# thien/stereo.vision

Hardware: AMD Instinct MI355X
Metric: Mpoints/sec disparity→3D at 1024×544; achieved HBM GB/s vs peak (higher is better)
Workload: dtype u8->f32; 1 GPU; configs[2]: 4096/GPU x 1024x544, step 1, dense fp32 XYZ (K1); frames_per_gpu=4096, global_frames=4096, H=544, W=1024, step=1, grid_points_per_frame=555489, parallelism=frame-sharded x1; one process

## Files before the change

stereo.vision_amd/csrc/kernels/resident.hip:

```cpp
#include "../svx_launch.h"

namespace svx {

constexpr int kRMaxChunks = 256;
constexpr int kRBins = 1000;
constexpr int kRDN = 32;
constexpr int kRDxStride = 33;
constexpr int kRDyOff = kRDN * kRDxStride;
constexpr int kRTxGroup = 20;
constexpr int kRTyOff = 64 * kRTxGroup;
constexpr int kRDeltaWords = kRTyOff + 32 > kRDyOff + kRDN ? kRTyOff + 32 : kRDyOff + kRDN;

__device__ __forceinline__ uint32_t pk_max16(uint32_t a, uint32_t b) {
    typedef unsigned short us2 __attribute__((ext_vector_type(2)));
    return __builtin_bit_cast(uint32_t, __builtin_elementwise_max(__builtin_bit_cast(us2, a), __builtin_bit_cast(us2, b)));
}


template <int STEP, int QP, bool LC>
struct RCfg {
    static constexpr int QPL = QP;
    static constexpr int CW = 3 * STEP;
};
template <int STEP>
// ... 537 lines not shown
        uint32_t cw[QPL][RCfg<STEP, QP, LC>::CW];
        r_load_bgr<STEP, QP, LC>(fbgr, r.g, p, cw);
        __syncthreads();
        uint32_t pos0;
        const uint32_t wtotal = r_stage_colours_sel<STEP, QP, LC>(keep, cw, wstage, sh.dump + tid, pos0);
        for (uint32_t j = lane; j < wtotal; j += kWave) {
            const uint32_t bin = r_bin_sel(wstage[j]);
            wstage[j] = (int64_t)hist[bin] > (int64_t)p.hist_thr ? 1u : 0u;
        }
        uint32_t pos = pos0;
#pragma unroll
        for (int b = 0; b < 4 * QPL; ++b) {
            if (keep & (1u << b)) {
                if (!wstage[pos]) keep &= ~(1u << b);
                ++pos;
            }
        }
    }
    uint64_t cnt = 0, inc;
    const auto add = [](uint32_t a, uint32_t b) { return a + b; };
    if constexpr (LC) {
        cnt = (uint64_t)__builtin_popcount(keep);
        inc = (uint64_t)wave_scan_dpp((uint32_t)cnt, add);
    } else {
#pragma unroll
        for (int i = 0; i < QPL; ++i) cnt += (uint64_t)__builtin_popcount((keep >> (4 * i)) & 0xF) << (16 * i);
        inc = (uint64_t)wave_scan_dpp((uint32_t)cnt, add) | ((uint64_t)wave_scan_dpp((uint32_t)(cnt >> 32), add) << 32);
    }
    if (lane == 63) sh.wtot[wave] = inc;
    __syncthreads();
    uint64_t wbase = 0, tot = 0;
#pragma unroll
    for (int w = 0; w < 4; ++w) {
        const uint64_t v = sh.wtot[w];
        wbase += (w < wave) ? v : 0ull;
        tot += v;
    }
    const uint64_t excl = wbase + inc - cnt;
    const uint32_t T = LC ? (uint32_t)tot
                          : (uint32_t)((tot >> 0) & 0xFFFF) + (uint32_t)((tot >> 16) & 0xFFFF) +
                                (uint32_t)((tot >> 32) & 0xFFFF) + (uint32_t)((tot >> 48) & 0xFFFF);
    if (tid < (int)(running - flushed)) sh.stage[(flushed + tid) & (stage_of<QP>() - 1)] = sh.red[tid];
    if (T > (uint32_t)stage_of<QP>() - (running - flushed)) {
        p2_write<STEP, QP, LC>(sh.stage, flushed, running, oX, oY, oZ, oPxy, p);
        flushed = running;
        __syncthreads();
    }
    uint32_t rowbase = running;
    uint32_t olc = running + (uint32_t)excl;
    const uint32_t tyl = (LC && narrow) ? dl[kRTyOff + (((uint32_t)max(r.g.gy[0], 0) * STEP) & 31u)] : 0u;
    uint32_t bxm = 0u, bym = 0u;
#pragma unroll
    for (int i = 0; i < QPL; ++i) {
        uint32_t o = LC ? olc : rowbase + (uint32_t)((excl >> (16 * i)) & 0xFFFF);
        rowbase += (uint32_t)((tot >> (16 * i)) & 0xFFFF);
        const uint32_t gy = (uint32_t)max(r.g.gy[i], 0), y = gy * STEP;
        uint32_t dv[4], bx[4], by[4];
#pragma unroll
        for (int k = 0; k < 4; ++k) dv[k] = r_d<STEP, QP, LC>(r.dw[i], k);
        if (narrow && LC) {
            const uint32_t x0 = 4u * (uint32_t)r.g.q[0];
            const uint4 tw = *reinterpret_cast<const uint4*>(dl + (x0 >> 4) * kRTxGroup + 4 * i);
            const uint32_t t4[4] = {tw.x, tw.y, tw.z, tw.w};
#pragma unroll
            for (int k = 0; k < 4; ++k) {
                const uint32_t dd = min(dv[k] - (uint32_t)dlo, (uint32_t)kRDN - 1);
                bx[k] = (t4[k] >> dd) & 1u;
                by[k] = (tyl >> dd) & 1u;
            }
        } else if (narrow) {
#pragma unroll
            for (int k = 0; k < 4; ++k) {
                const uint32_t dd = min(dv[k] - (uint32_t)dlo, (uint32_t)kRDN - 1);
                const uint32_t x = (uint32_t)(4 * r.g.q[i] + k) * STEP;
                bx[k] = (dl[dd * kRDxStride + (x >> 5)] >> (x & 31)) & 1u;
                by[k] = (dl[kRDyOff + dd] >> (y & 31)) & 1u;
            }
        } else {
#pragma unroll
            for (int k = 0; k < 4; ++k) {
                const uint32_t x = (uint32_t)(4 * r.g.q[i] + k) * STEP;
                const uint32_t xw = min(x >> 5, (uint32_t)p.dx_words - 1);
                bx[k] = (bf.dxbits[dv[k] * p.dx_words + xw] >> (x & 31)) & 1u;
                by[k] = (bf.dybits[dv[k] * p.dy_words + (y >> 5)] >> (y & 31)) & 1u;
            }
        }
#pragma unroll
        for (int k = 0; k < 4; ++k) {
            const uint32_t bit = (keep >> (4 * i + k)) & 1u;
            *(bit ? &sh.stage[o & (stage_of<QP>() - 1)] : sh.dump + tid) =
                rdesc(dv[k], gy, (uint32_t)(4 * r.g.q[i] + k), bx[k], by[k]);
            o += bit;
            if constexpr (RB) {
                bxm |= bx[k] << (4 * i + k);
                bym |= by[k] << (4 * i + k);
            }
        }
        olc = o;
    }
    if constexpr (RB) {
        static_assert(!RB || (LC && STEP == 1 && QPL == 4), "the road bitmap needs lane-contiguous step-1 quads");
        rb_mark(sh, keep, bxm, bym, r.g.gy[0], 4 * r.g.q[0], bf.rb_Wu);
    }
    if (PF && more) p2_load<STEP, QP, LC>(r, c + 1, tid, fdisp, sh.crange, bf, p, true, next_run, fkb);
    __syncthreads();
    running += T;
    const uint32_t upto = more ? (running & ~31u) : running;
    if (tid < (int)(running - upto)) sh.red[tid] = sh.stage[(upto + tid) & (stage_of<QP>() - 1)];
    if (upto > flushed) {
        p2_write<STEP, QP, LC>(sh.stage, flushed, upto, oX, oY, oZ, oPxy, p);
        flushed = upto;
    }
}

template <int QP>
struct FusedShared {
    uint32_t hist[kRBins];
    uint32_t dirty[maxchunks_of<QP>() / 32];
    uint64_t wtot[4];
    uint32_t red[32];
    uint32_t stage[stage_of<QP>()];
    uint32_t dump[256];
    alignas(16) uint32_t crange[maxchunks_of<QP>() * 4];
    uint32_t dlt[kRDeltaWords];
    uint32_t cany[8];
    uint32_t rring[8 * 32];
    uint32_t rwrap[32];
};
static_assert(sizeof(FusedShared<4>) <= 32768, "5 workgroups per CU (160 KiB LDS), as many as 93 VGPRs allow");

template <int STEP, int QP, bool LC>
__device__ __forceinline__ void chunk_keepable_bits(FusedShared<QP>& sh, const FramePlane* Lp, const RParams& p) {
    constexpr int per = RCfg<STEP, QP, LC>::QPL * 256;
    const int c = threadIdx.x;
    bool k = false;
    const FramePlane L = *Lp;
    if (c < p.nchunks && L.valid) {
        const int gy0 = fastdiv40(c * per, p.Q_m40);
        const int gy1 = fastdiv40(min((c + 1) * per, p.frame_quads) - 1, p.Q_m40);
        k = rows_keepable(L, gy0, gy1, p.Wg, STEP);
    }
    const uint64_t m = __ballot(k);
    if (lane_id() == 0) {
        sh.cany[2 * (c >> 6)] = (uint32_t)m;
        sh.cany[2 * (c >> 6) + 1] = (uint32_t)(m >> 32);
    }
}

template <int QP>
__device__ __forceinline__ bool chunk_any(const FusedShared<QP>& sh, int c) {
    return __builtin_amdgcn_readfirstlane((sh.cany[c >> 5] >> (c & 31)) & 1u) != 0;
}

template <int STEP, int QP, bool LC, bool PF1 = false>
__device__ __forceinline__ void frame_pass1(int frame, FusedShared<QP>& sh, const PipeBuffers& bf,
                                            const RLean& L, const FramePlane* Lp,
                                            const RParams& p) {
    constexpr int WREGION = 64 * RCfg<STEP, QP, LC>::QPL * 4;
    const int tid = threadIdx.x, lane = lane_id(), wave = tid >> 6;
    const uint8_t* fdisp = bf.disp + (int64_t)frame * p.frame_px;
    const uint8_t* fbgr = bf.bgr + (int64_t)frame * p.frame_px * 3;
    uint32_t* wstage = sh.stage + wave * WREGION;
    for (int i = tid; i < kRBins; i += 256) sh.hist[i] = 0;
    if (tid < maxchunks_of<QP>() / 32) sh.dirty[tid] = 0;
    chunk_keepable_bits<STEP, QP, LC>(sh, Lp, p);
    __syncthreads();
    uint32_t nvalid = 0, nkept = 0;
    uint16_t* fkb = bf.kbits + (int64_t)frame * p.nchunks * 256;
    const int n1 = ablated(p.ablate, 128) ? 0 : p.nchunks;
    if constexpr (PF1) {
        P1Regs<STEP, QP, LC> r1;
        if (n1 > 0) p1_load<STEP, QP, LC>(r1, 0, tid, fdisp, fbgr, p, false, chunk_any(sh, 0));
        for (int c = 0; c < n1; ++c) {
            P1Regs<STEP, QP, LC> cur = r1;
            const bool any = chunk_any(sh, c);
            const uint32_t keep = any ? r_keep1<STEP, QP, LC>(cur.dw, cur.g, L, Lp, p.Wg) : 0u;
            if (c + 1 < n1) p1_load<STEP, QP, LC>(r1, c + 1, tid, fdisp, fbgr, p, true, chunk_any(sh, c + 1));
            p1_chunk<STEP, QP, LC>(cur, c, sh.hist, sh.dirty, sh.crange, wstage, sh.dump + tid, p, nvalid, nkept,
                               any, fkb, keep);
        }
    } else {
        for (int c = 0; c < n1; ++c) {
            P1Regs<STEP, QP, LC> r1;
            const bool any = chunk_any(sh, c);
            p1_load<STEP, QP, LC>(r1, c, tid, fdisp, fbgr, p, false, any);
            const uint32_t keep = any ? r_keep1<STEP, QP, LC>(r1.dw, r1.g, L, Lp, p.Wg) : 0u;
            p1_chunk<STEP, QP, LC>(r1, c, sh.hist, sh.dirty, sh.crange, wstage, sh.dump + tid, p, nvalid, nkept, any, fkb,
                               keep);
        }
    }
    nvalid = wave_sum(nvalid);
    nkept = wave_sum(nkept);
    if (lane == 0) {
        sh.red[wave] = nvalid;
        sh.red[4 + wave] = nkept;
    }
    __syncthreads();
}

template <int STEP, int QP, bool LC, bool PF, bool RB>
__device__ __forceinline__ void frame_pass2(int frame, FusedShared<QP>& sh, const PipeBuffers& bf,
                                            const RLean& L, const FramePlane* Lp,
                                            const RParams& p) {
    constexpr int WREGION = 64 * RCfg<STEP, QP, LC>::QPL * 4;
    const int tid = threadIdx.x, wave = tid >> 6;
    const uint8_t* fdisp = bf.disp + (int64_t)frame * p.frame_px;
    const uint8_t* fbgr = bf.bgr + (int64_t)frame * p.frame_px * 3;
    uint32_t* wstage = sh.stage + wave * WREGION;
    float* oX = bf.ox + (int64_t)frame * bf.ofs;
    float* oY = bf.oy + (int64_t)frame * bf.ofs;
    float* oZ = bf.oz + (int64_t)frame * bf.ofs;
    uint32_t* oPxy = bf.pxy + (int64_t)frame * bf.cap;
    uint32_t running = 0, flushed = 0;
    const int n2 = ablated(p.ablate, 256) ? 0 : p.nchunks;
    const auto run = [&](int c) {
        const uint4 cr = *reinterpret_cast<const uint4*>(sh.crange + 4 * c);
        return c + 1 == n2 || (cr.x | cr.y | cr.z | cr.w) != 0u;
    };
    const uint16_t* fkb = bf.kbits + (int64_t)frame * p.nchunks * 256;
    uint32_t* frb = RB ? bf.rbits + (int64_t)frame * bf.rb_H * 32 : nullptr;
    int rflushed = 0;
    if constexpr (RB) {
        sh.rring[tid] = 0u;
        if (tid < 32) sh.rwrap[tid] = 0u;
        __syncthreads();
    }
    constexpr int RPC = RB ? 4 : 1;
    P2Regs<STEP, QP, LC> r2;
    r2.staged = false;
    if (PF && n2 > 0) p2_load<STEP, QP, LC>(r2, 0, tid, fdisp, sh.crange, bf, p, false, run(0), fkb);
    for (int c = 0; c < n2; ++c) {
        if (!PF) p2_load<STEP, QP, LC>(r2, c, tid, fdisp, sh.crange, bf, p, c > 0, run(c), fkb);
        if (!run(c)) {
            if (PF) p2_load<STEP, QP, LC>(r2, c + 1, tid, fdisp, sh.crange, bf, p, true, run(c + 1), fkb);
            if constexpr (RB) rb_flush(sh, frb, rflushed, RPC * (c + 1) - 1, bf.rb_H);
            continue;
        }
        p2_chunk<STEP, QP, LC, PF, RB>(r2, c, c + 1 < n2, sh.hist, sh.dirty, sh, wstage, fdisp, fbgr, L, Lp, bf, oX, oY,
                                       oZ, oPxy,
                                       running, flushed, c + 1 < n2 && run(c + 1), fkb, p);
        if constexpr (RB) {
            if (c + 1 < n2) {
                rb_flush(sh, frb, rflushed, RPC * (c + 1) - 1, bf.rb_H);
            } else {
                while (rflushed < bf.rb_H) rb_flush(sh, frb, rflushed, min(rflushed + 8, bf.rb_H), bf.rb_H);
            }
        }
    }
    if (tid == 0) bf.counts[4 * (int64_t)frame + 2] = running;
}

template <int STEP, int QP, bool LC, bool PF, bool PF1, bool RB>
__device__ __forceinline__ void fused_body(const PipeBuffers& bf, const RParams& p,
                                           FusedShared<QP>& sh) {
    const int tid = threadIdx.x;
    const int frame = blockIdx.x;
    const FramePlane* Lp = bf.planes + (int64_t)frame * bf.plane_stride;
    const RLean L{Lp->al32, Lp->bb32, Lp->b032, Lp->tn32, Lp->g32};
    if (const uint32_t us = ablate_field(p.ablate, 20, 0xFFFu); us && blockIdx.x < 5 * 256) {
        const uint64_t t0 = wall_clock64(), wait = (uint64_t)(blockIdx.x >> 8) * us * 100u;
        while (wall_clock64() - t0 < wait) __builtin_amdgcn_s_sleep(32);
    }
    frame_pass1<STEP, QP, LC, PF1>(frame, sh, bf, L, Lp, p);
    __builtin_amdgcn_s_setprio(2);
    uint32_t* gh = bf.hist + (int64_t)frame * kBins;
    for (int b = tid; b < kBins; b += 256) gh[b] = b < kRBins ? sh.hist[b] : 0u;
    if (tid == 0) {
        int64_t* cn = bf.counts + 4 * (int64_t)frame;
        cn[0] = (int64_t)sh.red[0] + sh.red[1] + sh.red[2] + sh.red[3];
        cn[1] = (int64_t)sh.red[4] + sh.red[5] + sh.red[6] + sh.red[7];
    }
    frame_pass2<STEP, QP, LC, PF, RB>(frame, sh, bf, L, Lp, p);
}

template <int STEP, int QP, bool LC, bool PF, bool PF1 = false, bool RB = false>
__global__ __launch_bounds__(256) __attribute__((amdgpu_waves_per_eu(5))) void resident_fused_kernel(PipeBuffers bf, RParams p) {
    __shared__ FusedShared<QP> sh;
    fused_body<STEP, QP, LC, PF, PF1, RB>(bf, p, sh);
}

bool resident_supported(const KParams& p) {
    return (p.step == 1 || p.step == 2) && p.pitch <= 2048 && p.Hg <= 2048 &&
           resident_chunks_per_frame(p, 4) <= kRMaxChunks && p.frame_px * 3 < (1ll << 31);
}

static bool resident_lane_quads(const KParams& kp) {
    const char* v = svx_knob("SVX_RES_LC");
    const bool on = !(v && v[0] == '0');
    return on && kp.step == 1 && kp.Q % 4 == 0 && kp.W % 16 == 0 && kp.frame_px % 16 == 0;
}

bool resident_road_bits_supported(const KParams& p) {
    return resident_supported(p) && p.step == 1 && p.W == 1024 && p.Q == 256 && p.H <= 1024 && p.Hg >= 1 &&
           resident_lane_quads(p);
}

static RParams resident_params(const KParams& kp, int qpl) {
    RParams p;
    p.W = kp.W;
    p.Wg = kp.Wg;
    p.Q = kp.Q;
    p.pitch = kp.pitch;
    p.frame_quads = kp.frame_quads;
    p.nchunks = resident_chunks_per_frame(kp, qpl);
    p.drow = 256 * qpl / kp.Q;
    p.dq = 256 * qpl % kp.Q;
    p.hist_thr = kp.hist_thr;
    p.dx_words = kp.dx_words;
    p.dy_words = kp.dy_words;
    p.ablate = kp.ablate;
    p.Q_m40 = kp.Q_m40;
    p.frame_px = kp.frame_px;
    p.B32 = kp.B32;
    p.fB32 = kp.fB32;
    p.cw_hi = kp.cw_hi;
    p.cw_lo = kp.cw_lo;
    p.ch_hi = kp.ch_hi;
    p.ch_lo = kp.ch_lo;
    return p;
}

__global__ void store_plane_kernel(FramePlane v, FramePlane* __restrict__ dst) {
    if (threadIdx.x == 0) *dst = v;
}

hipError_t launch_store_plane(const FramePlane& v, FramePlane* dst, hipStream_t s) {
    hipLaunchKernelGGL(store_plane_kernel, dim3(1), dim3(64), 0, s, v, dst);
    return hipGetLastError();
}

hipError_t launch_pipeline_resident(const KParams& kp, const PipeBuffers& b, int frames,
                                    bool prefetch, hipStream_t s, bool prefetch1, const char** kname) {
    if (frames <= 0) return hipSuccess;
    if (!resident_supported(kp) || !b.planes) return hipErrorInvalidValue;
    const dim3 grid(frames), block(256);
// ... 35 lines not shown
```

stereo.vision_amd/csrc/kernels/sgbm.hip:

```cpp
#include <hip/hip_runtime.h>
#include <stdint.h>

#include <algorithm>
#include <type_traits>
#include <cstdlib>

#include "../svx_device.h"
#include "../svx_sgbm.h"
#include "../svx_wave.h"

namespace svx {
namespace {

constexpr int kMaxCost = 32767;
constexpr int kInt16Min = -32768;

__device__ __forceinline__ int lo16(uint32_t v) { return (int)(int16_t)(v & 0xFFFF); }
__device__ __forceinline__ int hi16(uint32_t v) { return (int)(int16_t)(v >> 16); }
__device__ __forceinline__ uint32_t pack16(int a, int b) { return (uint32_t)(uint16_t)a | ((uint32_t)(uint16_t)b << 16); }
__device__ __forceinline__ int sat16(int v) { return v < kInt16Min ? kInt16Min : (v > kMaxCost ? kMaxCost : v); }
__device__ __forceinline__ bool out16(int v) { return v < kInt16Min || v > kMaxCost; }

__device__ __forceinline__ int wave_min_i32(int v) {
    return wave_readlane(wave_scan(v, 0x7fffffff, [](int a, int b) { return min(a, b); }), 63);
// ... 412 lines not shown
                pk_step(cw, st, k.P1, k.P2, q);
                (q2vol + o)[lane] = q_byte_pk(q);
            } else {
                int L0, L1;
                path_step(cw0, cw1, st, k.P1, k.P2, L0, L1);
                (l2vol + o)[lane] = pack16(L0, L1);
            }
        }
#pragma unroll
        for (int u = 0; u < U; ++u) {
            ca[u] = na[u];
            cr[u] = nr[u];
        }
    }
    if (__any(st.ovf()) && lane == 0) atomicOr(flags + f, 1u);
}

template <int SH2C, bool DQ>
__global__ __launch_bounds__(256) void sgbm_vertical_ring_kernel(SgbmK k, const uint32_t* __restrict__ hvol,
                                                                   uint32_t* __restrict__ cvol,
                                                                   uint32_t* __restrict__ l2vol,
                                                                   uint8_t* __restrict__ q2vol,
                                                                   uint32_t* __restrict__ flags, int frames) {
    constexpr int RS = 2 * SH2C + 1;
    const int wpb = blockDim.x >> 6;
    const int cols_blocks = (k.width1 + wpb - 1) / wpb;
    const int f = blockIdx.x / cols_blocks;
    const int xi = (blockIdx.x - f * cols_blocks) * wpb + wave_uniform_id();
    if (f >= frames || xi >= k.width1) return;
    const uint32_t lane = lane_id();
    const int H = k.H;
    const size_t rs = (size_t)k.width1 * 64;
    const size_t base = (size_t)f * H * rs + (size_t)xi * 64;
    const uint32_t rs32 = (uint32_t)rs;
    const __amdgpu_buffer_rsrc_t rh = wave_rsrc(hvol + base, (size_t)H * rs * 4),
                                 rcv = wave_rsrc(cvol + base, (size_t)H * rs * 4), rq2 = wave_rsrc(q2vol + base, (size_t)H * rs);
    const auto hrow = [&](int r) { return bld32(rh, lane * 4, (uint32_t)min(r, H - 1) * rs32 * 4); };
    uint32_t drop[RS];
    int c0 = 0, c1 = 0;
#pragma unroll
    for (int kk = 0; kk <= SH2C; ++kk) {
        const uint32_t h = hrow(kk);
        const int sc = kk == 0 ? SH2C + 1 : 1;
        c0 += lo16(h) * sc;
        c1 += hi16(h) * sc;
        if (kk == 0) {
#pragma unroll
            for (int u = 0; u <= SH2C + 1; ++u) drop[u] = h;
        } else if (kk < SH2C) {
            drop[kk + SH2C + 1] = h;
        }
    }
    std::conditional_t<DQ, PathPk, PathState> st;
    const bool upd_col = xi > 0;
    uint32_t add[RS];
#pragma unroll
    for (int u = 0; u < RS; ++u) add[u] = hrow(u + SH2C);
    const auto vstep = [&](int u, int y) {
        if (y > 0 && upd_col && y + SH2C < H) {
            c0 += lo16(add[u]) - lo16(drop[u]);
            c1 += hi16(add[u]) - hi16(drop[u]);
        }
        drop[u] = add[u];
        const int cw0 = (int)(int16_t)c0, cw1 = (int)(int16_t)c1;
        const uint32_t cw = pack16(cw0, cw1);
        bst32(cw, rcv, lane * 4, (uint32_t)y * rs32 * 4);
        if constexpr (DQ) {
            uint32_t q;
            pk_step(cw, st, k.P1, k.P2, q);
            bst8(q_byte_pk(q), rq2, lane, (uint32_t)y * rs32);
        } else {
            int L0, L1;
            path_step(cw0, cw1, st, k.P1, k.P2, L0, L1);
            (l2vol + base + (size_t)y * rs)[lane] = pack16(L0, L1);
        }
    };
    int y0 = 0;
    for (; y0 + RS <= H; y0 += RS) {
        uint32_t nadd[RS];
#pragma unroll
        for (int u = 0; u < RS; ++u) nadd[u] = hrow(y0 + RS + u + SH2C);
#pragma unroll
        for (int u = 0; u < RS; ++u) vstep(u, y0 + u);
#pragma unroll
        for (int u = 0; u < RS; ++u) add[u] = nadd[u];
    }
#pragma unroll
    for (int u = 0; u < RS; ++u)
        if (y0 + u < H) vstep(u, y0 + u);
    if (__any(st.ovf()) && lane == 0) atomicOr(flags + f, 1u);
}

template <bool DQ>
__global__ __launch_bounds__(256) void sgbm_diag_kernel(SgbmK k, const uint32_t* __restrict__ cvol,
                                                          uint32_t* __restrict__ l1vol, uint32_t* __restrict__ l3vol,
                                                          uint8_t* __restrict__ q1vol, uint8_t* __restrict__ q3vol,
                                                          uint32_t* __restrict__ flags, int frames) {
    const int wpb = blockDim.x >> 6;
    const int npaths = k.width1 + k.H - 1;
    const int per_frame = 2 * npaths;
    const int gw = blockIdx.x * wpb + wave_uniform_id();
    const int f = gw / per_frame;
    if (f >= frames) return;
    int p = gw - f * per_frame;
    const int dir = p >= npaths;
    p -= dir * npaths;
    int xi, y;
    if (p < k.width1) {
        xi = p;
        y = 0;
    } else {
        xi = dir ? k.width1 - 1 : 0;
        y = p - k.width1 + 1;
    }
    const int len = min(k.H - y, dir ? xi + 1 : k.width1 - xi);
    const uint32_t lane = lane_id();
    const size_t rs = (size_t)k.width1 * 64;
    const size_t a0 = (size_t)f * k.H * rs + (size_t)y * rs + (size_t)xi * 64;
    const size_t step = dir ? rs - 64 : rs + 64;
    uint32_t* out = dir ? l3vol : l1vol;
    uint8_t* qout = dir ? q3vol : q1vol;
    const size_t span = (size_t)(len - 1) * step + 64;
    const __amdgpu_buffer_rsrc_t rc = wave_rsrc(cvol + a0, span * 4), rq = wave_rsrc(qout + a0, span);
    const uint32_t st32 = (uint32_t)step;
    const auto cell = [&](int t) { return bld32(rc, lane * 4, (uint32_t)min(t, len - 1) * st32 * 4); };
    std::conditional_t<DQ, PathPk, PathState> st;
    constexpr int U = kSgPf;
    uint32_t cc[U];
#pragma unroll
    for (int u = 0; u < U; ++u) cc[u] = cell(u);
    for (int t0 = 0; t0 < len; t0 += U) {
        uint32_t nc[U];
#pragma unroll
        for (int u = 0; u < U; ++u) nc[u] = cell(t0 + U + u);
#pragma unroll
        for (int u = 0; u < U; ++u) {
            const int t = t0 + u;
            if (t >= len) break;
            const size_t o = a0 + (size_t)t * step;
            if constexpr (DQ) {
                uint32_t q;
                pk_step(cc[u], st, k.P1, k.P2, q);
                bst8(q_byte_pk(q), rq, lane, (uint32_t)t * st32);
            } else {
                int L0, L1;
                path_step(lo16(cc[u]), hi16(cc[u]), st, k.P1, k.P2, L0, L1);
                (out + o)[lane] = pack16(L0, L1);
            }
        }
#pragma unroll
        for (int u = 0; u < U; ++u) cc[u] = nc[u];
    }
    if (__any(st.ovf()) && lane == 0) atomicOr(flags + f, 1u);
}


__host__ __device__ constexpr size_t sgbm_row_lds_per_wave(int W) { return ((size_t)6 * W + 3) & ~(size_t)3; }

template <bool DQ>
__global__ __launch_bounds__(256) void sgbm_row_kernel(SgbmK k, const uint32_t* __restrict__ cvol,
                                                         uint32_t* __restrict__ l1p, const uint32_t* __restrict__ l2vol,
                                                         const uint32_t* __restrict__ l3vol,
                                                         uint8_t* __restrict__ q0vol, const uint8_t* __restrict__ q1vol,
                                                         const uint8_t* __restrict__ q2vol,
                                                         const uint8_t* __restrict__ q3vol, int16_t* __restrict__ d16,
                                                         uint32_t* __restrict__ flags, int frames) {
    constexpr int U = kSgPf;
    extern __shared__ uint32_t rsm32[];
    const int wpb = blockDim.x >> 6, wave = wave_uniform_id();
    const int gw = blockIdx.x * wpb + wave;
    const int f = gw / k.H, y = gw - f * k.H;
    if (f >= frames) return;
    const int W = k.W;
    const uint32_t lane = lane_id();
    uint32_t* d2key = rsm32 + wave * (sgbm_row_lds_per_wave(W) / 4);
    int16_t* disp1 = reinterpret_cast<int16_t*>(d2key + W);
    const int INVALID = -kSgScale;
    for (int x = lane; x < W; x += 64) {
        disp1[x] = (int16_t)INVALID;
        d2key[x] = ~0u;
    }
    wave_lds_sync();
    const size_t rs = (size_t)k.width1 * 64;
    const size_t rb = ((size_t)f * k.H + y) * rs;
    const int n = k.width1;
    const auto at = [&](auto* vol, int xi) { return vol + rb + (size_t)xi * 64; };
    const __amdgpu_buffer_rsrc_t rc = wave_rsrc(cvol + rb, rs * 4), rq0 = wave_rsrc(q0vol + rb, rs),
                                 rq1 = wave_rsrc(q1vol + rb, rs), rq2 = wave_rsrc(q2vol + rb, rs),
                                 rq3 = wave_rsrc(q3vol + rb, rs);
    std::conditional_t<DQ, PathPk, PathState> sa, sb;
    {
        uint32_t cc[U], ca[U], cb[U], ce[U];
        const auto load = [&](int xi, uint32_t& c, uint32_t& a, uint32_t& b, uint32_t& e) {
            xi = min(xi, n - 1);
            if constexpr (DQ) {
                c = bld32(rc, lane * 4, (uint32_t)xi * 256);
            } else {
                c = at(cvol, xi)[lane];
                a = at(l1p, xi)[lane];
                b = at(l2vol, xi)[lane];
                e = at(l3vol, xi)[lane];
            }
        };
#pragma unroll
        for (int u = 0; u < U; ++u) load(u, cc[u], ca[u], cb[u], ce[u]);
        for (int x0 = 0; x0 < n; x0 += U) {
            uint32_t nc[U], na[U], nb[U], ne[U];
#pragma unroll
            for (int u = 0; u < U; ++u) load(x0 + U + u, nc[u], na[u], nb[u], ne[u]);
#pragma unroll
            for (int u = 0; u < U; ++u) {
                const int xi = x0 + u;
                if (xi >= n) break;
                if constexpr (DQ) {
                    uint32_t q;
                    pk_step(cc[u], sa, k.P1, k.P2, q);
                    bst8(q_byte_pk(q), rq0, lane, (uint32_t)xi * 64);
                } else {
                    int L0, L1;
                    path_step(lo16(cc[u]), hi16(cc[u]), sa, k.P1, k.P2, L0, L1);
                    const uint32_t pv = pack16(sat16(L0 + lo16(ca[u]) + lo16(cb[u]) + lo16(ce[u])),
                                               sat16(L1 + hi16(ca[u]) + hi16(cb[u]) + hi16(ce[u])));
                    __builtin_nontemporal_store(pv, at(l1p, xi) + lane);
                }
            }
#pragma unroll
            for (int u = 0; u < U; ++u) {
                cc[u] = nc[u];
                ca[u] = na[u];
                cb[u] = nb[u];
                ce[u] = ne[u];
            }
        }
    }
    {
        const int d0 = 2 * lane;
        uint32_t cc[U], cp[U];
        const auto load = [&](int j, uint32_t& c, uint32_t& pp) {
            const int xi = max(n - 1 - j, 0);
            if constexpr (DQ) {
                const uint32_t so = (uint32_t)xi * 64;
                c = bld32(rc, lane * 4, so * 4, true);
                pp = bld8(rq0, lane, so, true) | bld8(rq1, lane, so, true) << 8 | bld8(rq2, lane, so, true) << 16 |
                     bld8(rq3, lane, so, true) << 24;
            } else {
                c = at(cvol, xi)[lane];
                pp = at(l1p, xi)[lane];
            }
        };
#pragma unroll
        for (int u = 0; u < U; ++u) load(u, cc[u], cp[u]);
        for (int j0 = 0; j0 < n; j0 += U) {
            uint32_t nc[U], np[U];
#pragma unroll
            for (int u = 0; u < U; ++u) load(j0 + U + u, nc[u], np[u]);
            int gkey = -1, gnum = 0, gdv = 1;
#pragma unroll
            for (int u = 0; u < U; ++u) {
                const int xi = n - 1 - (j0 + u);
                if (xi < 0) break;
                int L0, L1, lm;
                uint32_t Lpk = 0;
                int P0, P1;
                if constexpr (DQ) {
                    uint32_t q;
                    Lpk = pk_l(cc[u], sb, k.P1, k.P2, q, lm);
                    L0 = lo16(Lpk);
                    L1 = hi16(Lpk);
                    P0 = sat16(4 * lo16(cc[u]) - (int)__builtin_amdgcn_sad_u8(cp[u] & 0x0F0F0F0Fu, 0u, 0u));
                    P1 = sat16(4 * hi16(cc[u]) - (int)__builtin_amdgcn_sad_u8((cp[u] >> 4) & 0x0F0F0F0Fu, 0u, 0u));
                } else {
                    lm = path_l(lo16(cc[u]), hi16(cc[u]), sb, k.P1, k.P2, L0, L1);
                    P0 = lo16(cp[u]);
                    P1 = hi16(cp[u]);
                }
                const int S0 = sat16(P0 + L0), S1 = sat16(P1 + L1);
                const int key = min(((S0 + 32768) << 7) | d0, ((S1 + 32768) << 7) | (d0 + 1));
                int wm, kmin;
                wave_min2_i32(lm, key, wm, kmin);
                if constexpr (DQ)
                    pk_commit(sb, cc[u], Lpk, wm);
                else
                    path_commit(sb, L0, L1, lm, wm);
                const int minS = (kmin >> 7) - 32768, best = kmin & 127;
                bool write = minS != kMaxCost;
                if (k.uniq > 0) {
                    const bool bad = (S0 * (100 - k.uniq) < minS * 100 && abs(best - d0) > 1) ||
                                     (S1 * (100 - k.uniq) < minS * 100 && abs(best - d0 - 1) > 1);
                    if (__any(bad)) write = false;
                }
                int num = 0, dv = 1;
                if (write && best > 0 && best < kSgD - 1) {
                    const uint32_t spk = pack16(S0, S1);
                    const uint32_t wm = (uint32_t)__builtin_amdgcn_readlane((int)spk, (best - 1) >> 1);
                    const uint32_t wp = (uint32_t)__builtin_amdgcn_readlane((int)spk, (best + 1) >> 1);
                    const int Sm = (best - 1) & 1 ? hi16(wm) : lo16(wm);
                    const int Sp = (best + 1) & 1 ? hi16(wp) : lo16(wp);
                    const int den = max(Sm + Sp - 2 * minS, 1);
                    num = (Sm - Sp) * kSgScale + den;
                    dv = den * 2;
                }
                if (write && lane == (uint32_t)u) {
                    gkey = kmin;
                    gnum = num;
                    gdv = dv;
                }
// ... 234 lines not shown
    t[threadIdx.x] = lut ? lut[threadIdx.x] : (uint8_t)threadIdx.x;
    __syncthreads();
    const int64_t per = (px + gridDim.x - 1) / gridDim.x;
    const int f = blockIdx.y;
    const int64_t p0 = blockIdx.x * per, p1 = min(px, p0 + per);
    const uint8_t* src = bgr + (size_t)f * px * 3;
    for (int64_t p = p0 + threadIdx.x; p < p1; p += blockDim.x) {
        const uint8_t* c = src + 3 * p;
        const int g = (t[c[0]] * 1868 + t[c[1]] * 9617 + t[c[2]] * 4899 + (1 << 13)) >> 14;
        grey[(size_t)f * px + p] = (uint8_t)g;
        atomicAdd(&h[g], 1u);
    }
    __syncthreads();
    if (h[threadIdx.x]) atomicAdd(hist + f * 256 + threadIdx.x, h[threadIdx.x]);
}

__global__ __launch_bounds__(256) void equalize_kernel(uint8_t* __restrict__ grey, int64_t px,
                                                         const uint32_t* __restrict__ hist) {
    __shared__ uint8_t lut[256];
    const int f = blockIdx.y;
    const uint32_t* h = hist + f * 256;
    if (threadIdx.x == 0) {
        int i = 0;
        while (i < 255 && !h[i]) ++i;
        if ((int64_t)h[i] == px) {
            for (int j = 0; j < 256; ++j) lut[j] = (uint8_t)i;
        } else {
            const float scale = 255.f / (float)(px - (int64_t)h[i]);
            int64_t sum = 0;
            lut[i] = 0;
            for (int j = i + 1; j < 256; ++j) {
                sum += h[j];
                const float v = __fmul_rn((float)sum, scale);
                const int r = (int)rintf(v);
                lut[j] = (uint8_t)(r < 0 ? 0 : r > 255 ? 255 : r);
            }
            for (int j = 0; j < i; ++j) lut[j] = 0;
        }
    }
    __syncthreads();
    uint8_t* g = grey + (size_t)f * px;
    for (int64_t p = (int64_t)blockIdx.x * blockDim.x + threadIdx.x; p < px; p += (int64_t)gridDim.x * blockDim.x)
        g[p] = lut[g[p]];
}

__global__ void synth_pair_kernel(uint8_t* __restrict__ left, uint8_t* __restrict__ right, int H, int W, int frames,
                                  int64_t first) {
    const int64_t i = (int64_t)blockIdx.x * blockDim.x + threadIdx.x;
    const int64_t px = (int64_t)H * W;
    const int64_t f = i / px;
    if (f >= frames) return;
    const int p = (int)(i - f * px);
    const int y = p / W, x = p - y * W;
    const int D = sgbm_pair_disparity(y);
    left[i] = sgbm_pair_texture(first + f, H, y, x);
    right[i] = sgbm_pair_texture(first + f, H, y, x + D);
}

__global__ void synth_bgr_pair_kernel(uint8_t* __restrict__ left, uint8_t* __restrict__ right, int H, int W,
                                      int frames, int64_t first) {
    const int64_t i = (int64_t)blockIdx.x * blockDim.x + threadIdx.x;
    const int64_t px = (int64_t)H * W;
    const int64_t f = i / px;
    if (f >= frames) return;
    const int p = (int)(i - f * px);
    const int y = p / W, x = p - y * W;
    const int D = sgbm_pair_disparity(y);
#pragma unroll
    for (int side = 0; side < 2; ++side) {
        const int u = side ? x + D : x;
        const int t = sgbm_pair_texture(first + f, H, y, u);
        const int j = sgbm_pair_texture(first + f + 0x4000000000ll, H, y, u);
        uint8_t* o = (side ? right : left) + 3 * i;
        o[0] = (uint8_t)t;
        o[1] = (uint8_t)min(255, t + (j & 31));
        o[2] = (uint8_t)max(0, t - ((j >> 3) & 31));
    }
}

__global__ __launch_bounds__(256) void copy_bgr_region_kernel(const uint8_t* __restrict__ src, int Hp, int Wp,
                                                              uint8_t* __restrict__ dst, int H, int W, int Wu,
                                                              const uint8_t* __restrict__ lut) {
    __shared__ uint8_t t[256];
    t[threadIdx.x] = lut ? lut[threadIdx.x] : (uint8_t)threadIdx.x;
    __syncthreads();
    const int row = blockIdx.x, f = blockIdx.y;
    const uint8_t* s = src + ((int64_t)f * Hp + row) * Wp * 3;
    uint8_t* d = dst + ((int64_t)f * H + row) * W * 3;
    for (int b = threadIdx.x; b < 3 * Wu; b += blockDim.x) d[b] = t[s[b]];
}

}

hipError_t launch_synth_bgr_pair(uint8_t* left, uint8_t* right, int H, int W, int frames, int64_t first,
                                 hipStream_t s) {
    const int64_t n = (int64_t)frames * H * W;
    hipLaunchKernelGGL(synth_bgr_pair_kernel, dim3((unsigned)((n + 255) / 256)), dim3(256), 0, s, left, right, H, W,
                       frames, first);
    return hipGetLastError();
}

hipError_t launch_copy_bgr_region(const uint8_t* src, int Hp, int Wp, uint8_t* dst, int H, int W, int Wu, int frames,
                                  hipStream_t s, const uint8_t* lut) {
    if (frames <= 0 || H <= 0) return hipSuccess;
    if (H > Hp || Wu > Wp || Wu > W) return hipErrorInvalidValue;
    hipLaunchKernelGGL(copy_bgr_region_kernel, dim3((unsigned)H, (unsigned)frames), dim3(256), 0, s, src, Hp, Wp, dst,
                       H, W, Wu, lut);
    return hipGetLastError();
}

bool sgbm_supported(const SgbmK& k) {
    const size_t frame_vol = (size_t)(k.H + 1) * ((size_t)k.width1 * 64 + 64) * sizeof(uint32_t);
    return k.width1 > k.SW2 && k.W <= 2048 && k.H >= 1 && k.SW2 >= 0 && k.SW2 <= 31 && frame_vol < 0x7FFFFFFFu;
}

size_t sgbm_volume_bytes(const SgbmK& k) { return (size_t)k.H * k.width1 * kSgD * sizeof(int16_t); }

hipError_t launch_sgbm_compute(const SgbmK& k, const uint8_t* left, const uint8_t* right, int frames,
                               const SgbmScratch& s, hipStream_t st) {
    const int H = k.H;
    hipError_t e = hipMemsetAsync(s.flags, 0, sizeof(uint32_t) * frames, st);
    if (e != hipSuccess) return e;
    const char* hr = svx_knob("SVX_SGBM_HRING");
#ifdef SVX_DIAG
    const char* ha = svx_knob("SVX_SGBM_HSUM_ABLATE");
    const int habl = ha && *ha ? std::atoi(ha) : 0;
#else
    constexpr int habl = 0;
#endif
    if (k.SW2 == 10 && !(hr && hr[0] == '0')) {
        if (habl == 0)
            hipLaunchKernelGGL(sgbm_hsum_ring_kernel<10>, dim3(frames * H), dim3(256), 28 * (size_t)k.W, st, k, left,
                               right, s.hl1, frames);
#ifdef SVX_DIAG
        else if (habl == 1)
            hipLaunchKernelGGL((sgbm_hsum_ring_kernel<10, 1>), dim3(frames * H), dim3(256), 28 * (size_t)k.W, st, k,
                               left, right, s.hl1, frames);
        else if (habl == 2)
            hipLaunchKernelGGL((sgbm_hsum_ring_kernel<10, 2>), dim3(frames * H), dim3(256), 28 * (size_t)k.W, st, k,
                               left, right, s.hl1, frames);
        else
            hipLaunchKernelGGL((sgbm_hsum_ring_kernel<10, 3>), dim3(frames * H), dim3(256), 28 * (size_t)k.W, st, k,
                               left, right, s.hl1, frames);
#endif
    } else {
        const size_t lds1 = sizeof(uint32_t) * (5 * (size_t)k.W + 4 * (2 * k.SW2 + 1) * 64);
        hipLaunchKernelGGL(sgbm_hsum_kernel, dim3(frames * H), dim3(256), lds1, st, k, left, right, s.hl1, frames);
    }
    const int cb = (k.width1 + 3) / 4;
    const int paths = 2 * (k.width1 + H - 1) * frames;
    const size_t lds4 = sgbm_row_lds_per_wave(k.W) * 4;
    const char* vr = svx_knob("SVX_SGBM_VRING");
    const bool vring = k.SH2 == 10 && !(vr && vr[0] == '0');
    const char* dqv = svx_knob("SVX_SGBM_DQ");
    const bool dq = k.P1 >= 0 && k.P2 <= 15 && !(dqv && dqv[0] == '0');
    const size_t qb = (size_t)frames * H * k.width1 * 64;
    uint8_t* q0 = reinterpret_cast<uint8_t*>(s.l3);
    uint8_t* q1 = q0 + qb;
    uint8_t* q2 = q1 + qb;
    uint8_t* q3 = q2 + qb;
#define SVX_SGBM_WALKS(DQ)                                                                                        \
    if (vring)                                                                                                    \
        hipLaunchKernelGGL((sgbm_vertical_ring_kernel<10, DQ>), dim3(frames * cb), dim3(256), 0, st, k, s.hl1,   \
                           s.c, s.l2, q2, s.flags, frames);                                                       \
    else                                                                                                          \
        hipLaunchKernelGGL(sgbm_vertical_kernel<DQ>, dim3(frames * cb), dim3(256), 0, st, k, s.hl1, s.c, s.l2,   \
                           q2, s.flags, frames);                                                                  \
    hipLaunchKernelGGL(sgbm_diag_kernel<DQ>, dim3((paths + 3) / 4), dim3(256), 0, st, k, s.c, s.hl1, s.l3, q1,   \
                       q3, s.flags, frames);                                                                      \
    hipLaunchKernelGGL(sgbm_row_kernel<DQ>, dim3((frames * H + 3) / 4), dim3(256), lds4, st, k, s.c, s.hl1,      \
                       s.l2, s.l3, q0, q1, q2, q3, s.raw, s.flags, frames)
    if (dq) {
        SVX_SGBM_WALKS(true);
    } else {
        SVX_SGBM_WALKS(false);
    }
#undef SVX_SGBM_WALKS
    if (frames > 65535) return hipErrorInvalidValue;
    hipLaunchKernelGGL(sgbm_median3_kernel, dim3((unsigned)((k.frame_px + 255) / 256), (unsigned)frames), dim3(256), 0,
                       st, k.H, k.W, k.frame_px, s.raw, s.d16, frames);
    return hipGetLastError();
}

hipError_t launch_speckle_scale(const SgbmK& k, int frames, const SgbmScratch& s, uint8_t* out, int16_t* filt,
                                hipStream_t st) {
    const int64_t n = (int64_t)frames * k.frame_px;
    if (frames > 65535) return hipErrorInvalidValue;
    const unsigned rows = (unsigned)((frames * k.H + 3) / 4);
    hipLaunchKernelGGL(sgbm_cc_rows_kernel, dim3(rows), dim3(256), 0, st, k, s.d16, s.parent, frames);
    hipLaunchKernelGGL(sgbm_cc_union_kernel, dim3((unsigned)((k.frame_px + 255) / 256), (unsigned)frames), dim3(256), 0,
                       st, k, s.d16, s.parent, frames);
    hipError_t e = hipMemsetAsync(s.size, 0, sizeof(int32_t) * n, st);
    if (e != hipSuccess) return e;
    hipLaunchKernelGGL(sgbm_cc_count_kernel, dim3(rows), dim3(256), 0, st, k, s.d16, s.parent, s.size, frames);
    hipLaunchKernelGGL(sgbm_out_rows_kernel, dim3(rows), dim3(256), 0, st, k, s.d16, s.parent, s.size, out, filt,
                       frames);
    return hipGetLastError();
}

hipError_t launch_lut(const uint8_t* in, int64_t n, const uint8_t* lut, uint8_t* out, hipStream_t s) {
    if (n <= 0) return hipSuccess;
    const int64_t blocks = std::min<int64_t>((n + 1023) / 1024, 8192);
    hipLaunchKernelGGL(lut_kernel, dim3((unsigned)blocks), dim3(256), 0, s, in, n, lut, out);
    return hipGetLastError();
}

hipError_t launch_grey_equalize(const uint8_t* bgr, int64_t px, int frames, uint8_t* grey, uint32_t* hist,
                                hipStream_t s, const uint8_t* lut) {
    hipError_t e = hipMemsetAsync(hist, 0, sizeof(uint32_t) * 256 * frames, s);
    if (e != hipSuccess) return e;
    const unsigned bx = (unsigned)std::min<int64_t>((px + 4095) / 4096, 256);
    hipLaunchKernelGGL(grey_hist_kernel, dim3(bx, frames), dim3(256), 0, s, bgr, px, frames, grey, hist, lut);
    hipLaunchKernelGGL(equalize_kernel, dim3(bx, frames), dim3(256), 0, s, grey, px, hist);
    return hipGetLastError();
}

hipError_t launch_synth_pair(uint8_t* left, uint8_t* right, int H, int W, int frames, int64_t first, hipStream_t s) {
    const int64_t n = (int64_t)frames * H * W;
    hipLaunchKernelGGL(synth_pair_kernel, dim3((unsigned)((n + 255) / 256)), dim3(256), 0, s, left, right, H, W,
                       frames, first);
    return hipGetLastError();
}

}
```

Before: 537,000 Mpoints/s.

## Batch runs of non-keepable chunks into a lightweight unrolled disparity-count pass

Pass 1 now treats chunks with no keepable rows separately. It finds runs of such chunks from the cany bitmask and processes each run with a lean routine that only loads disparity and counts valid points. That routine keeps 8 loads in flight. The main per-chunk loop now jumps straight to the next keepable chunk, and crange is zeroed up front for the chunks it skips. This cuts per-chunk overhead (BGR loads, histogram and staging work) on dead chunks and adds memory-level parallelism, at the cost of more registers (U×QPL×STEP disparity words) and more control flow.

```diff
diff --git a/stereo.vision_amd/csrc/kernels/resident.hip b/stereo.vision_amd/csrc/kernels/resident.hip
--- a/stereo.vision_amd/csrc/kernels/resident.hip
+++ b/stereo.vision_amd/csrc/kernels/resident.hip
@@ -713,6 +713,60 @@
     return __builtin_amdgcn_readfirstlane((sh.cany[c >> 5] >> (c & 31)) & 1u) != 0;
 }
 
+constexpr int kRunU = 8;
+
+template <int QP>
+__device__ __forceinline__ int next_chunk(const FusedShared<QP>& sh, int c, int last, bool any) {
+    const uint32_t x = any ? 0u : ~0u;
+    int w = c >> 5;
+    uint32_t m = (sh.cany[w] ^ x) & (~0u << (c & 31));
+    while (m == 0u && 32 * (w + 1) <= last) m = sh.cany[++w] ^ x;
+    const int e = m ? 32 * w + (int)__builtin_ctz(m) : last;
+    return __builtin_amdgcn_readfirstlane(min(e, last));
+}
+
+template <int K>
+struct RunSlot {
+    static constexpr int value = K;
+};
+template <int K, int N, class F>
+__device__ __forceinline__ void run_unrolled(const F& f) {
+    if constexpr (K < N) {
+        f(RunSlot<K>{});
+        run_unrolled<K + 1, N>(f);
+    }
+}
+
+template <int STEP, int QP, bool LC>
+__device__ __forceinline__ void p1_skip_run(int c0, int c1, int tid, const uint8_t* fdisp, const RParams& p,
+                                            uint32_t& nvalid) {
+    constexpr int QPL = RCfg<STEP, QP, LC>::QPL, U = kRunU;
+    uint32_t dw[U][QPL][STEP];
+    RQuads<STEP, QP, LC> gi, gu;
+    r_geometry<STEP, QP, LC>(c0, tid, p, gi);
+    gu = gi;
+    run_unrolled<0, U>([&](auto k) {
+        if (c0 + k.value < c1) {
+            if (k.value > 0) r_geometry_next<STEP, QP, LC>(c0 + k.value, tid, p, gi);
+            r_load_disp<STEP, QP, LC>(fdisp, gi, p, dw[k.value]);
+        }
+    });
+#pragma unroll 1
+    for (int base = c0; base < c1; base += U) {
+        run_unrolled<0, U>([&](auto k) {
+            const int c = base + k.value;
+            if (c < c1) {
+                nvalid += r_nvalid<STEP, QP, LC>(dw[k.value], gu, p);
+                if (c + U < c1) {
+                    r_geometry_next<STEP, QP, LC>(c + U, tid, p, gi);
+                    r_load_disp<STEP, QP, LC>(fdisp, gi, p, dw[k.value]);
+                }
+                r_geometry_next<STEP, QP, LC>(c + 1, tid, p, gu);
+            }
+        });
+    }
+}
+
 template <int STEP, int QP, bool LC, bool PF1 = false>
 __device__ __forceinline__ void frame_pass1(int frame, FusedShared<QP>& sh, const PipeBuffers& bf,
                                             const RLean& L, const FramePlane* Lp,
@@ -724,24 +778,39 @@
     uint32_t* wstage = sh.stage + wave * WREGION;
     for (int i = tid; i < kRBins; i += 256) sh.hist[i] = 0;
     if (tid < maxchunks_of<QP>() / 32) sh.dirty[tid] = 0;
+    for (int i = tid; i < 4 * p.nchunks; i += 256) sh.crange[i] = 0u;
     chunk_keepable_bits<STEP, QP, LC>(sh, Lp, p);
     __syncthreads();
     uint32_t nvalid = 0, nkept = 0;
     uint16_t* fkb = bf.kbits + (int64_t)frame * p.nchunks * 256;
     const int n1 = ablated(p.ablate, 128) ? 0 : p.nchunks;
+    const int last = n1 - 1;
+    const auto taken = [&](int c) { return c < last && !chunk_any(sh, c) ? next_chunk(sh, c, last, true) : c; };
+    const auto skip_runs = [&]() {
+        for (int c = next_chunk(sh, 0, last, false); c < last;) {
+            const int c1 = next_chunk(sh, c, last, true);
+            p1_skip_run<STEP, QP, LC>(c, c1, tid, fdisp, p, nvalid);
+            c = next_chunk(sh, c1, last, false);
+        }
+    };
     if constexpr (PF1) {
         P1Regs<STEP, QP, LC> r1;
-        if (n1 > 0) p1_load<STEP, QP, LC>(r1, 0, tid, fdisp, fbgr, p, false, chunk_any(sh, 0));
-        for (int c = 0; c < n1; ++c) {
+        int c = n1 > 0 ? taken(0) : 0;
+        if (n1 > 0) p1_load<STEP, QP, LC>(r1, c, tid, fdisp, fbgr, p, false, chunk_any(sh, c));
+        skip_runs();
+        while (c < n1) {
             P1Regs<STEP, QP, LC> cur = r1;
             const bool any = chunk_any(sh, c);
             const uint32_t keep = any ? r_keep1<STEP, QP, LC>(cur.dw, cur.g, L, Lp, p.Wg) : 0u;
-            if (c + 1 < n1) p1_load<STEP, QP, LC>(r1, c + 1, tid, fdisp, fbgr, p, true, chunk_any(sh, c + 1));
+            const int cn = c + 1 < n1 ? taken(c + 1) : n1;
+            if (cn < n1) p1_load<STEP, QP, LC>(r1, cn, tid, fdisp, fbgr, p, cn == c + 1, chunk_any(sh, cn));
             p1_chunk<STEP, QP, LC>(cur, c, sh.hist, sh.dirty, sh.crange, wstage, sh.dump + tid, p, nvalid, nkept,
                                any, fkb, keep);
+            c = cn;
         }
     } else {
-        for (int c = 0; c < n1; ++c) {
+        skip_runs();
+        for (int c = n1 > 0 ? taken(0) : 0; c < n1; c = c + 1 < n1 ? taken(c + 1) : n1) {
             P1Regs<STEP, QP, LC> r1;
             const bool any = chunk_any(sh, c);
             p1_load<STEP, QP, LC>(r1, c, tid, fdisp, fbgr, p, false, any);
```

New measurement: 522,600 Mpoints/s. 0.973x the previous value.

## Walk SGBM diagonal paths with wraparound so each wave covers a fixed-length path

Applied to the files above, without the earlier changes.

Adds a diagonal aggregation kernel where each wave starts at one column and walks down all H rows. At the image edge it wraps to the opposite column and resets the path state. This replaces the old per-diagonal walks, which had variable lengths (2*(width1+H-1) paths per frame), with width1 equal-length walks per direction. The goal is balanced wave work, fewer waves, and prefetch that is not broken by early-exit tails. The cost is a reset branch on every step and modulo-style index updates. The new kernel is on by default and can be disabled with SVX_SGBM_DIAG=0.

```diff
diff --git a/stereo.vision_amd/csrc/kernels/sgbm.hip b/stereo.vision_amd/csrc/kernels/sgbm.hip
--- a/stereo.vision_amd/csrc/kernels/sgbm.hip
+++ b/stereo.vision_amd/csrc/kernels/sgbm.hip
@@ -588,6 +588,90 @@
         for (int u = 0; u < U; ++u) cc[u] = nc[u];
     }
     if (__any(st.ovf()) && lane == 0) atomicOr(flags + f, 1u);
+}
+
+template <bool DQ, int DIR>
+__device__ __forceinline__ void sgbm_diag_wrap_walk(const SgbmK& k, const uint32_t* __restrict__ cvol,
+                                                    void* __restrict__ ovol, uint32_t* __restrict__ flags, int f,
+                                                    int x0) {
+    const int n = k.width1, H = k.H;
+    const uint32_t lane = lane_id();
+    const size_t cells = (size_t)H * n;
+    const size_t fb = (size_t)f * cells * 64;
+    const __amdgpu_buffer_rsrc_t rc = wave_rsrc(cvol + fb, cells * 256);
+    const __amdgpu_buffer_rsrc_t ro = DQ ? wave_rsrc(static_cast<uint8_t*>(ovol) + fb, cells * 64)
+                                         : wave_rsrc(static_cast<uint32_t*>(ovol) + fb, cells * 256);
+    const auto next = [&](int x) { return DIR ? (x == 0 ? n - 1 : x - 1) : (x == n - 1 ? 0 : x + 1); };
+    const int edge = DIR ? n - 1 : 0;
+    std::conditional_t<DQ, PathPk, PathState> st;
+    constexpr int U = kSgPf;
+    int xl = x0, rl = 0;
+    const int rlast = (H - 1) * n;
+    const auto cell = [&]() {
+        const uint32_t c = bld32(rc, lane * 4, (uint32_t)(rl + xl) * 256);
+        xl = next(xl);
+        rl = min(rl + n, rlast);
+        return c;
+    };
+    int xs = x0, rs = 0;
+    const auto dstep = [&](uint32_t c) {
+        if (xs == edge) {
+            if constexpr (DQ) {
+                st.p = 0;
+            } else {
+                st.p0 = 0;
+                st.p1 = 0;
+            }
+            st.pmin = 0;
+        }
+        const uint32_t o = (uint32_t)(rs + xs);
+        if constexpr (DQ) {
+            uint32_t q;
+            pk_step(c, st, k.P1, k.P2, q);
+            bst8(q_byte_pk(q), ro, lane, o * 64);
+        } else {
+            int L0, L1;
+            path_step(lo16(c), hi16(c), st, k.P1, k.P2, L0, L1);
+            bst32(pack16(L0, L1), ro, lane * 4, o * 256);
+        }
+        xs = next(xs);
+        rs += n;
+    };
+    uint32_t cc[U];
+#pragma unroll
+    for (int u = 0; u < U; ++u) cc[u] = cell();
+    int t0 = 0;
+    for (; t0 + U <= H; t0 += U) {
+        uint32_t nc[U];
+#pragma unroll
+        for (int u = 0; u < U; ++u) nc[u] = cell();
+#pragma unroll
+        for (int u = 0; u < U; ++u) dstep(cc[u]);
+#pragma unroll
+        for (int u = 0; u < U; ++u) cc[u] = nc[u];
+    }
+#pragma unroll
+    for (int u = 0; u < U; ++u)
+        if (t0 + u < H) dstep(cc[u]);
+    if (__any(st.ovf()) && lane == 0) atomicOr(flags + f, 1u);
+}
+
+template <bool DQ>
+__global__ __launch_bounds__(256) void sgbm_diag_wrap_kernel(SgbmK k, const uint32_t* __restrict__ cvol,
+                                                               uint32_t* __restrict__ l1vol,
+                                                               uint32_t* __restrict__ l3vol,
+                                                               uint8_t* __restrict__ q1vol,
+                                                               uint8_t* __restrict__ q3vol,
+                                                               uint32_t* __restrict__ flags, int frames) {
+    const int wgf = (k.width1 + 1) >> 1;
+    const int f = blockIdx.x / wgf;
+    const int w = wave_uniform_id();
+    const int x0 = (blockIdx.x - f * wgf) * 2 + (w & 1);
+    if (f >= frames || w >= 4 || x0 >= k.width1) return;
+    if (w >> 1)
+        sgbm_diag_wrap_walk<DQ, 1>(k, cvol, DQ ? (void*)q3vol : (void*)l3vol, flags, f, x0);
+    else
+        sgbm_diag_wrap_walk<DQ, 0>(k, cvol, DQ ? (void*)q1vol : (void*)l1vol, flags, f, x0);
 }
 
 
@@ -1128,6 +1212,8 @@
     const size_t lds4 = sgbm_row_lds_per_wave(k.W) * 4;
     const char* vr = svx_knob("SVX_SGBM_VRING");
     const bool vring = k.SH2 == 10 && !(vr && vr[0] == '0');
+    const char* dg = svx_knob("SVX_SGBM_DIAG");
+    const bool dwrap = !(dg && dg[0] == '0');
     const char* dqv = svx_knob("SVX_SGBM_DQ");
     const bool dq = k.P1 >= 0 && k.P2 <= 15 && !(dqv && dqv[0] == '0');
     const size_t qb = (size_t)frames * H * k.width1 * 64;
@@ -1142,8 +1228,12 @@
     else                                                                                                          \
         hipLaunchKernelGGL(sgbm_vertical_kernel<DQ>, dim3(frames * cb), dim3(256), 0, st, k, s.hl1, s.c, s.l2,   \
                            q2, s.flags, frames);                                                                  \
-    hipLaunchKernelGGL(sgbm_diag_kernel<DQ>, dim3((paths + 3) / 4), dim3(256), 0, st, k, s.c, s.hl1, s.l3, q1,   \
-                       q3, s.flags, frames);                                                                      \
+    if (dwrap)                                                                                                    \
+        hipLaunchKernelGGL(sgbm_diag_wrap_kernel<DQ>, dim3(frames * ((k.width1 + 1) / 2)), dim3(256), 0, st, k,  \
+                           s.c, s.hl1, s.l3, q1, q3, s.flags, frames);                                            \
+    else                                                                                                          \
+        hipLaunchKernelGGL(sgbm_diag_kernel<DQ>, dim3((paths + 3) / 4), dim3(256), 0, st, k, s.c, s.hl1, s.l3,   \
+                           q1, q3, s.flags, frames);                                                              \
     hipLaunchKernelGGL(sgbm_row_kernel<DQ>, dim3((frames * H + 3) / 4), dim3(256), lds4, st, k, s.c, s.hl1,      \
                        s.l2, s.l3, q0, q1, q2, q3, s.raw, s.flags, frames)
     if (dq) {
```

After: 524,700 Mpoints/s before, 523,200 Mpoints/s after. No clear change (-0.3%).
